# voidstrike/FPSG

Hardware: AMD Instinct MI355X
Metric: episodes/sec (+ Chamfer-kernel HBM GB/s in roofline.hbm), 2048-pt clouds, 224x224 images; episode = fwd + Chamfer + bwd, step = E episodes + all-reduce + Adam (higher is better)
Workload: dtype f32

## Files before the change

### fpsg_amd/_hip.py

```python
from __future__ import annotations

import ctypes
import os
import threading

import torch

_HERE = os.path.dirname(os.path.abspath(__file__))
LIB_PATH = os.environ.get("FPSG_HIP_LIB") or os.path.join(_HERE, "libfpsg_hip.so")

_c_f32p = ctypes.c_void_p
_c_i32p = ctypes.c_void_p
_c_int = ctypes.c_int
_c_stream = ctypes.c_void_p

SIGNATURES = {
    "fpsg_version": [],
    "fpsg_last_error": [],
    "fpsg_chamfer_fwd": [_c_f32p, _c_f32p, _c_int, _c_int, _c_int,
                         _c_f32p, _c_i32p, _c_f32p, _c_i32p, _c_stream],
    "fpsg_chamfer_bwd": [_c_f32p, _c_f32p, _c_i32p, _c_i32p, _c_f32p, _c_f32p,
                         _c_int, _c_int, _c_int, _c_f32p, _c_f32p, _c_stream],
    "fpsg_chamfer_losses": [_c_f32p, _c_f32p, _c_int, _c_int, _c_int, _c_int, ctypes.c_float, ctypes.c_float, _c_f32p,
                            _c_stream],
# ... 44 lines not shown
                                 _c_stream],
    "fpsg_sinkhorn_grad_workspace_floats": [_c_int, _c_int, _c_int],
    "fpsg_sinkhorn_divergence_grad": [_c_f32p, _c_f32p, _c_int, _c_int, _c_int, ctypes.c_void_p, _c_int, _c_f32p, _c_f32p,
                                      _c_f32p, _c_f32p, _c_stream],
    "fpsg_dec1_tiles": [_c_int],
    "fpsg_dec1_fits": [_c_int, _c_int, _c_int],
    "fpsg_dec1_fwd": [_c_f32p, _c_f32p, _c_int, _c_int, _c_f32p, _c_f32p, _c_f32p, _c_f32p, _c_f32p, _c_int, _c_int,
                      _c_int, _c_int, _c_int, ctypes.c_float, _c_f32p, _c_f32p, _c_f32p, _c_f32p, _c_stream],
    "fpsg_dec1_bwd": [_c_f32p, _c_f32p, _c_f32p, _c_int, _c_int, _c_f32p, _c_f32p, _c_int, _c_int, _c_int, _c_int,
                      _c_int, _c_f32p, _c_f32p, _c_f32p, _c_f32p, _c_f32p, _c_stream],
    "fpsg_dec1_fwd_ld": [_c_f32p, _c_int, _c_f32p, _c_int, _c_int, _c_f32p, _c_int, _c_f32p, _c_f32p, _c_f32p, _c_f32p, _c_int,
                         _c_int, _c_int, _c_int, _c_int, ctypes.c_float, _c_f32p, _c_int, _c_f32p, _c_f32p, _c_f32p,
                         _c_stream],
    "fpsg_dec1_bwd_ld": [_c_f32p, _c_int, _c_f32p, _c_int, _c_f32p, _c_int, _c_int, _c_f32p, _c_int, _c_f32p, _c_int, _c_int,
                         _c_int, _c_int, _c_int, _c_int, _c_f32p, _c_f32p, _c_f32p, _c_f32p, _c_f32p, _c_stream],
    "fpsg_bn_act_rows_fwd": [_c_f32p, _c_int, ctypes.POINTER(ctypes.c_int), ctypes.POINTER(ctypes.c_int), _c_int,
                             _c_f32p, _c_f32p, _c_f32p, _c_int, ctypes.c_float, _c_int, ctypes.c_float, _c_f32p,
                             _c_f32p, _c_f32p, _c_stream],
    "fpsg_bn_act_rows_bwd": [_c_f32p, _c_int, ctypes.POINTER(ctypes.c_int), ctypes.POINTER(ctypes.c_int), _c_int,
                             _c_f32p, _c_f32p, _c_f32p, _c_int, _c_int, ctypes.c_float, _c_f32p, _c_f32p, _c_f32p,
                             _c_f32p, _c_stream],
    "fpsg_bn_workspace_floats": [_c_int, _c_int, _c_int],
    "fpsg_bn_act_fwd": [_c_f32p, _c_f32p, _c_f32p, _c_f32p, _c_f32p, _c_f32p, ctypes.c_float, _c_int, _c_int, _c_int, _c_int,
                        ctypes.c_float, _c_int, ctypes.c_float, _c_f32p, _c_f32p, _c_f32p, _c_f32p, _c_f32p,
                        _c_stream],
    "fpsg_bn_act_bwd": [_c_f32p, _c_f32p, _c_f32p, _c_f32p, _c_int, _c_int, _c_int, _c_int, _c_int,
                        ctypes.c_float, _c_f32p, _c_f32p, _c_f32p, _c_f32p, _c_f32p, _c_f32p, _c_stream],
    "fpsg_bn_act_bwd_coef": [_c_f32p, _c_f32p, _c_f32p, _c_f32p, _c_int, _c_int, _c_int, _c_int, _c_int, ctypes.c_float,
                             _c_f32p, _c_f32p, _c_f32p, _c_f32p, _c_stream],
    "fpsg_bn_act_bwd_parts": [_c_f32p, _c_f32p, _c_f32p, _c_f32p, _c_int, _c_int, _c_int, _c_int, _c_int,
# ... 134 lines not shown
                         ctypes.POINTER(ctypes.c_float), _c_int, ctypes.c_void_p, ctypes.c_void_p, _c_f32p, _c_i32p,
                         _c_f32p, ctypes.c_void_p, ctypes.c_size_t, _c_stream],
    "fpsg_mesh_render_materials_workspace_bytes": [_c_int, _c_int, _c_int, _c_int, _c_int, _c_int, _c_int],
    "fpsg_mesh_render_materials": [_c_f32p, _c_int, _c_i32p, _c_int, _c_i32p, _c_f32p, ctypes.POINTER(ctypes.c_float),
                                   _c_int, ctypes.POINTER(ctypes.c_int32), _c_int, ctypes.c_void_p, ctypes.c_longlong,
                                   _c_f32p, _c_int, _c_int, _c_int, _c_int, ctypes.c_float,
                                   ctypes.POINTER(ctypes.c_float), _c_int, ctypes.c_void_p, ctypes.c_void_p, _c_f32p,
                                   _c_i32p, _c_f32p, ctypes.c_void_p, ctypes.c_size_t, _c_stream],
    "fpsg_points_render_workspace_bytes": [_c_int, _c_int, _c_int, _c_int, _c_int],
    "fpsg_points_render": [_c_f32p, ctypes.c_void_p, _c_int, _c_int, _c_f32p, _c_int, _c_int, _c_int, _c_int,
                           ctypes.c_float, ctypes.c_float, ctypes.POINTER(ctypes.c_float), _c_int, ctypes.c_void_p,
                           ctypes.c_void_p, _c_f32p, _c_i32p, _c_f32p, ctypes.c_void_p, ctypes.c_size_t, _c_stream],
}
_RESTYPES = {"fpsg_last_error": ctypes.c_char_p, "fpsg_grad_norm_workspace_bytes": ctypes.c_size_t,
"fpsg_chamfer_workspace_bytes": ctypes.c_size_t,
             "fpsg_sinkhorn_workspace_floats": ctypes.c_size_t,
             "fpsg_sinkhorn_grad_workspace_floats": ctypes.c_size_t,
             "fpsg_knn_workspace_floats": ctypes.c_size_t,
             "fpsg_bn_workspace_floats": ctypes.c_size_t, "fpsg_bn_pool_workspace_floats": ctypes.c_size_t, "fpsg_bn_max_workspace_floats": ctypes.c_size_t, "fpsg_bn_max_dz_offset": ctypes.c_size_t, "fpsg_conv_first_dw_workspace_floats": ctypes.c_size_t, "fpsg_emd_workspace_floats": ctypes.c_size_t, "fpsg_emd_exact_workspace_floats": ctypes.c_size_t, "fpsg_emd_cross_workspace_bytes": ctypes.c_size_t, "fpsg_occupancy_grid_workspace_bytes": ctypes.c_size_t, "fpsg_fps_workspace_bytes": ctypes.c_size_t, "fpsg_max_bwd_scatter_workspace_floats": ctypes.c_size_t,
             "fpsg_wino_dw_fused_workspace_floats": ctypes.c_size_t, "fpsg_gemm_split_workspace_floats": ctypes.c_size_t, "fpsg_gemm_split_packed_a_bytes": ctypes.c_size_t, "fpsg_edgeconv_stats_ws_floats": ctypes.c_size_t,
             "fpsg_repulsion_workspace_bytes": ctypes.c_size_t,
             "fpsg_expansion_workspace_bytes": ctypes.c_size_t,
             "fpsg_uniform_workspace_bytes": ctypes.c_size_t,
             "fpsg_swd_workspace_bytes": ctypes.c_size_t,
             "fpsg_mesh_cdf_workspace_bytes": ctypes.c_size_t,
             "fpsg_mesh_render_workspace_bytes": ctypes.c_size_t,
             "fpsg_mesh_render_materials_workspace_bytes": ctypes.c_size_t,
             "fpsg_points_render_workspace_bytes": ctypes.c_size_t}

_lib = None
# ... 53 lines not shown
```

### fpsg_amd/csrc/bnact.hip

```cpp
#include <algorithm>
#include <initializer_list>

#include "fpsg_common.h"

namespace fpsg {
namespace {

constexpr int kBnThreads = 256;
constexpr int kBnSeg = 4096;
constexpr int kBnSlices = 64;
constexpr int kBnU = kBnSeg / 4 / kBnThreads;

enum BnAct { kActNone = 0, kActRelu = 1, kActLeaky = 2 };

template <int ACT>
__device__ __forceinline__ float act_fwd(float z, float slope) {
  if (ACT == kActRelu) return z > 0.0f ? z : 0.0f;
  if (ACT == kActLeaky) return z > 0.0f ? z : z * slope;
  return z;
}
template <int ACT>
__device__ __forceinline__ float act_grad(float z, float slope) {
  if (ACT == kActRelu) return z > 0.0f ? 1.0f : 0.0f;
  if (ACT == kActLeaky) return z > 0.0f ? 1.0f : slope;
// ... 255 lines not shown
  for (int off = 32; off >= 1; off >>= 1) a += __shfl_down(a, off, 64);
  if (threadIdx.x == 0) dpb[c] = (float)a;
}

constexpr int kBnSmallMax = 16384;

constexpr int kBnMaxSegs = 4;
struct BnSegs {
  int ld;
  int off[kBnMaxSegs], len[kBnMaxSegs];
  int staged[kBnMaxSegs];
  int tpr_log2[kBnMaxSegs];
  int stat_stride;
};

template <int MODE, int ACT>
__global__ __launch_bounds__(kBnThreads) void bn_small_kernel(
    const float* __restrict__ x, const float* __restrict__ dy, const float* __restrict__ gamma,
    const float* __restrict__ beta, const float* __restrict__ pb, int N, int C, BnSegs segs, int training, float eps,
    float slope, float* __restrict__ out, float* __restrict__ chan, float* __restrict__ batch_mean,
    float* __restrict__ batch_var_unbiased, float* __restrict__ dgamma, float* __restrict__ dbeta,
    float* __restrict__ dpb, float* __restrict__ run_mean, float* __restrict__ run_var, float momentum) {
  const int sgi = blockIdx.y;
  const int L = segs.len[sgi], ld = segs.ld, staged = segs.staged[sgi], tpr_log2 = segs.tpr_log2[sgi];
  x += segs.off[sgi];
  out += segs.off[sgi];
  if (MODE == 1) dy += segs.off[sgi];
  chan += (size_t)sgi * 4 * C;
  if (batch_mean) batch_mean += (size_t)sgi * segs.stat_stride;
  if (batch_var_unbiased) batch_var_unbiased += (size_t)sgi * segs.stat_stride;
  if (MODE == 1) {
    dgamma += (size_t)sgi * C;
    dbeta += (size_t)sgi * C;
    if (dpb) dpb += (size_t)sgi * C;
  }
  extern __shared__ __attribute__((aligned(16))) float stage[];
  __shared__ float red[8];
  __shared__ float bc[4];
  const int c = blockIdx.x;
  const float b = pb ? pb[c] : 0.0f;
  const double count = (double)N * (double)L;
// ... 97 lines not shown
        chan[c] = bc[0]; chan[C + c] = bc[1]; chan[2 * C + c] = bc[2]; chan[3 * C + c] = bc[3];
        const float unbiased = (float)(count > 1.0 ? var * count / (count - 1.0) : var);
        if (batch_mean) batch_mean[c] = (float)mean;
        if (batch_var_unbiased) batch_var_unbiased[c] = unbiased;
        if (run_mean && momentum >= 0.0f) {
          run_mean[c] = fma_rn(momentum, (float)mean, (1.0f - momentum) * run_mean[c]);
          run_var[c] = fma_rn(momentum, unbiased, (1.0f - momentum) * run_var[c]);
        }
      } else {
        dbeta[c] = a0; dgamma[c] = a1;
        const double k2 = training ? -(double)sc * a1 * rs / count : 0.0;
        bc[0] = sc; bc[1] = (float)k2;
        bc[2] = training ? (float)(-(double)sc * a0 / count - k2 * mu) : 0.0f;
      }
    }
    __syncthreads();
    if (MODE == 0) { sc = bc[0]; sh = bc[1]; }
  } else {
    if (threadIdx.x == 0) { bc[0] = sc; bc[1] = 0.0f; bc[2] = 0.0f; }
    __syncthreads();
  }
  const float k1 = bc[0], k2 = bc[1], k3 = bc[2];
  float acc = 0.0f, unused = 0.0f;
  for (int n = n0; n < N; n += rpi) {
    const size_t base = ((size_t)n * C + c) * ld;
    if (vec) {
      const v4f* __restrict__ xp = reinterpret_cast<const v4f*>(x + base);
      const v4f* __restrict__ gp = reinterpret_cast<const v4f*>(MODE == 1 ? dy + base : x + base);
      v4f* __restrict__ op = reinterpret_cast<v4f*>(out + base);
      for (int e = e0; e < L4; e += tpr) {
// ... 645 lines not shown
  g.ld = ld;
  for (int i = 0; i < nseg; ++i) {
    FPSG_REQUIRE(seg_len[i] > 0 && seg_len[i] <= kBnSmallMax && seg_off[i] >= 0 && seg_off[i] + seg_len[i] <= ld,
                 FPSG_E_SHAPE, "%s: segment %d = [%d, +%d) does not fit a row of %d (a segment holds at most %d)", fn, i,
                 seg_off[i], seg_len[i], ld, kBnSmallMax);
    FPSG_REQUIRE((seg_off[i] & 3) == 0, FPSG_E_ALIGN, "%s: segment offset %d must be a multiple of 4", fn, seg_off[i]);
    for (int j = 0; j < i; ++j)
      FPSG_REQUIRE(seg_off[i] >= seg_off[j] + seg_len[j] || seg_off[j] >= seg_off[i] + seg_len[i], FPSG_E_SHAPE,
                   "%s: segments %d and %d overlap", fn, j, i);
    small_segment(g, i, 1, seg_off[i], seg_len[i], 1, backward);
  }
  return 0;
}

}
}

extern "C" size_t fpsg_bn_workspace_floats(int N, int C, int L) {
  if (N <= 0 || C <= 0 || L <= 0) return 0;
  return fpsg::plain_workspace(N, C, L).floats;
}

extern "C" int fpsg_bn_act_fwd(const float* x, const float* pre_bias, const float* gamma, const float* beta,
                               float* running_mean, float* running_var, float momentum, int N, int C, int L,
                               int training, float eps, int act, float slope, float* y, float* chan,
                               float* batch_mean, float* batch_var_unbiased, float* ws, fpsg_stream_t stream) {
  using namespace fpsg;
  const char* fn = "fpsg_bn_act_fwd";
  int rc = check_dims(fn, N, C, L, act);
  if (rc) return rc;
// ... 248 lines not shown
```

### fpsg_amd/csrc/decoder.hip

```cpp
#include "fpsg_common.h"

namespace fpsg {
namespace {

constexpr int kD1Waves = 8;
constexpr int kD1Threads = 64 * kD1Waves;
constexpr int kD1ChPerWave = 4;
constexpr int kD1Tile = kD1Waves * kD1ChPerWave;
constexpr int kD1MaxBP = 8192;
constexpr size_t kD1MaxLds = 160 * 1024;

inline size_t dec1_lds_bytes(int B, int P, bool bwd) {
  return ((size_t)3 * B * P + (size_t)kD1Tile * B + (bwd ? (size_t)kD1Waves * 64 * 12 : 0)) * sizeof(float);
}

__device__ __forceinline__ double wave_sum_f64(double v) {
#pragma unroll
  for (int m = 1; m < 64; m <<= 1) {
    const unsigned long long u = (unsigned long long)__double_as_longlong(v);
    unsigned lo = (unsigned)u, hi = (unsigned)(u >> 32);
    lo = (unsigned)__shfl_xor((int)lo, m, 64);
    hi = (unsigned)__shfl_xor((int)hi, m, 64);
    v += __longlong_as_double((long long)(((unsigned long long)hi << 32) | lo));
  }
// ... 291 lines not shown
    }
  }
}

inline int dec1_check(const char* fn, int G, int D, int B, int P, int ldw, int wofs, bool bwd) {
  FPSG_REQUIRE(G > 0 && D > 0 && B > 0 && P > 0, FPSG_E_SHAPE, "%s: G,D,B,P must be positive (got %d,%d,%d,%d)", fn, G,
               D, B, P);
  FPSG_REQUIRE(P % 4 == 0 && P <= 256 && ((P / 4) & (P / 4 - 1)) == 0, FPSG_E_SHAPE,
               "%s: P = %d must be 4 x a power of two, at most 256 (lanes of 4 points, a cloud = one lane group)", fn, P);
  FPSG_REQUIRE((long)B * P <= kD1MaxBP, FPSG_E_LIMIT, "%s: B*P = %ld exceeds %d (the patch's points live in LDS)", fn,
               (long)B * P, kD1MaxBP);
  FPSG_REQUIRE(dec1_lds_bytes(B, P, bwd) <= kD1MaxLds, FPSG_E_LIMIT,
               "%s: B = %d, P = %d need %zu bytes of LDS, more than the %zu of a CU", fn, B, P, dec1_lds_bytes(B, P, bwd),
               kD1MaxLds);
  FPSG_REQUIRE(G <= 65535 && wofs >= 0 && wofs + 3 <= ldw, FPSG_E_SHAPE, "%s: bad G / weight columns", fn);
  return 0;
}

}
}

extern "C" int fpsg_dec1_tiles(int D) { return (D + fpsg::kD1Tile - 1) / fpsg::kD1Tile; }

extern "C" int fpsg_dec1_fits(int B, int P, int bwd) {
  return fpsg::dec1_check("fpsg_dec1_fits", 1, 1, B, P, 3, 0, bwd != 0) == 0;
}

extern "C" int fpsg_dec1_fwd_ld(const float* hlat, int ld_hlat, const float* w, int ldw, int wofs, const float* pts, int ld_pts,
                                const float* gamma, const float* beta, const float* running_mean,
                                const float* running_var, int G, int D, int B, int P, int training, float eps,
// ... 57 lines not shown
                                       hipFuncAttributeMaxDynamicSharedMemorySize, (int)lds_bytes);
    if (e != hipSuccess) { set_error("fpsg_dec1_bwd: %s", hipGetErrorString(e)); return (int)e; }
  }
  hipLaunchKernelGGL(kern, dim3((unsigned)fpsg_dec1_tiles(D), (unsigned)G), dim3(kD1Threads), lds_bytes,
                     static_cast<hipStream_t>(stream), a, dout, chan, dhlat, dw, dpts_part, dgamma, dbeta);
  return launch_status("fpsg_dec1_bwd");
}

extern "C" int fpsg_dec1_bwd(const float* dout, const float* hlat, const float* w, int ldw, int wofs,
                             const float* pts, const float* chan, int G, int D, int B, int P, int training,
                             float* dhlat, float* dw, float* dpts_part, float* dgamma, float* dbeta,
                             fpsg_stream_t stream) {
  return fpsg_dec1_bwd_ld(dout, B * P, hlat, B, w, ldw, wofs, pts, B * P, chan, G, D, B, P, training, 0, dhlat, dw,
                          dpts_part, dgamma, dbeta, stream);
}
```

### fpsg_amd/csrc/fpsg_common.h

```cpp
#pragma once
#include <hip/hip_runtime.h>
#include <stdint.h>
#include <stdio.h>

#include "../../include/fpsg_hip.h"

namespace fpsg {

void set_error(const char* fmt, ...);

inline bool misaligned4(const void* p) { return (reinterpret_cast<uintptr_t>(p) & 3u) != 0; }

inline int launch_status(const char* what) {
  hipError_t e = hipGetLastError();
  if (e != hipSuccess) {
    set_error("%s: %s", what, hipGetErrorString(e));
    return static_cast<int>(e);
  }
  return 0;
}

#define FPSG_REQUIRE_PTR(p)                                   \
  do {                                                        \
    if ((p) == nullptr) {                                     \
// ... 88 lines not shown
```

### fpsg_amd/point_cloud_net.py

```python
from __future__ import annotations

import os

import torch
import torch.nn as nn
import torch.nn.functional as F

from . import bn_counters
from .fused_bn import batch_norm_act, batch_norm_act_rows, bn_act
from .pointnet import PointNetfeat
from .utils import get_template


def get_activation(argument: str):
    table = {
        "relu": F.relu,
        "sigmoid": torch.sigmoid,
        "softplus": F.softplus,
        "logsigmoid": F.logsigmoid,
        "softsign": F.softsign,
        "tanh": torch.tanh,
    }
    if argument not in table:
        raise ValueError(f"Invalid activation: {argument}")
# ... 313 lines not shown
            for i, Bi in enumerate(batches):
                part = torch.empty((G, T, 3, Bi * P), dtype=torch.float32, device=dev)
                rc = lib.fpsg_dec1_bwd_ld(_hip.ptr(dout) + 4 * b0 * P, M, _hip.ptr(hlat) + 4 * b0, B, _hip.ptr(w1), K, L,
                                          _hip.ptr(pts) + 4 * b0 * P, M, _hip.ptr(chan[i]), G, D, Bi, P, 1,
                                          1 if i else 0, _hip.ptr(dhlat) + 4 * b0, _hip.ptr(gw), _hip.ptr(part),
                                          _hip.ptr(dgamma), _hip.ptr(dbeta), _hip.stream_of(x))
                _hip.check(rc, "fpsg_dec1_bwd_ld")
                torch.sum(part, dim=1, out=gpts[:, :, b0 * P:(b0 + Bi) * P])
                b0 += Bi
        torch.bmm(dhlat, x.unsqueeze(0).expand(G, B, L), out=gw[..., :L])
        gb = dhlat.sum(dim=2, keepdim=True)
        gx = torch.matmul(dhlat.reshape(G * D, B).t(), w1.reshape(G * D, K)[:, :L])
        return gw, gb, gx, gpts, dgamma, dbeta, None, None, None


class _StackFrozen(torch.autograd.Function):

    @staticmethod
    def forward(ctx, key, *tensors):
        from . import winograd
        cache = winograd.frozen_cache()
        full_key = ("stack", key) + tuple(t.data_ptr() for t in tensors)
        if cache is not None and full_key in cache:
            return cache[full_key].detach()
        out = torch.stack([t.detach() for t in tensors])
        if cache is not None:
            cache[full_key] = out
            return out.detach()
        return out

# ... 311 lines not shown
        else:
            cols = []
            for i, b in enumerate(batches):
                if grids[i] is not None:
                    g = torch.stack([t for per_cluster in grids[i] for t in per_cluster])
                else:
                    g = torch.empty((G, b, dim, P), dtype=torch.float32, device=x.device)
                    g = g.uniform_(0, 1, generator=generator) if square else g.normal_(0, 1, generator=generator)
                cols.append(g.permute(0, 2, 1, 3).reshape(G, g.size(2), b * P))
            h = torch.cat(cols, dim=2)

        defs = [c.deformer for c in clusters]
        w, b = pack["d1"]
        h = _group_batch_norm_rows(torch.bmm(w, h), [d.bn1 for d in defs], R, act, pack["dbn1"], b.reshape(-1), seg_lens)
        w, b = pack["d2"]
        h = _group_batch_norm_rows(torch.bmm(w, h), [d.bn2 for d in defs], R, act, pack["dbn2"], b.reshape(-1), seg_lens)
        w, b = pack["d3"]
        pts = torch.tanh(torch.baddbmm(b, w, h))

        nodes = [n for c in clusters for n in c.node_pool]
        w1, b1 = pack["n1"]
        if w1.size(2) - self.conf.raw_dim != L:
            raise ValueError(f"PCDecoder: hidden size {L} does not match the first layer ({w1.size(2) - self.conf.raw_dim} latent columns)")
        bn1s = [n.bn1 for n in nodes]
        gamma, beta = pack["nbn1"]
        h, stats = _DecoderLayer1Pair.apply(w1, b1, x, pts, gamma, beta, bn1s[0].eps, P, batches)
        with torch.no_grad():
            _update_running_calls(bn1s, 1, stats)
        w, b = pack["n2"]
        h = _group_batch_norm_rows(_bmm_wide(w, h), [n.bn2 for n in nodes], 1, act, pack["nbn2"], b.reshape(-1), seg_lens)
        w, b = pack["n3"]
        h = _group_batch_norm_rows(_bmm_wide(w, h), [n.bn3 for n in nodes], 1, act, pack["nbn3"], b.reshape(-1), seg_lens)
        w, b = pack["n4"]
        out = torch.tanh(torch.baddbmm(b, w, h))
        return out.view(G, 3, B, P).permute(2, 0, 3, 1).reshape(B, G * P, 3).contiguous()

    def pack_parameters(self):
        if not self.batched:
            return None
        cache = key = None
        if not torch.is_grad_enabled() and os.environ.get("FPSG_EVAL_PACK_CACHE", "1") != "0":
            from . import winograd
            cache = winograd.frozen_cache()
            first = next(self.parameters())
            key = ("decoder_pack", id(self), first.data_ptr(), first.device)
            if cache is not None and key in cache:
                return cache[key]
        pack = self._build_pack()
        if cache is not None and not (first.is_cuda and torch.cuda.is_current_stream_capturing()):
# ... 44 lines not shown
        act = clusters[0].deformer.activation
        if grid is None:
            dim = clusters[0].template[0].dim
            if type(clusters[0].template[0]).__name__ == "SquareTemplate":
                g = torch.empty((G, B, dim, P), dtype=torch.float32, device=x.device).uniform_(0, 1, generator=generator)
            else:
                g = torch.empty((G, B, dim, P), dtype=torch.float32, device=x.device).normal_(0, 1, generator=generator)
        else:
            g = torch.stack([t for per_cluster in grid for t in per_cluster])
        h = g.permute(0, 2, 1, 3).reshape(G, g.size(2), B * P)

        defs = [c.deformer for c in clusters]
        w, b = pack["d1"]
        h = _group_batch_norm(torch.bmm(w, h), [d.bn1 for d in defs], R, act, pack["dbn1"], b.reshape(-1))
        w, b = pack["d2"]
        h = _group_batch_norm(torch.bmm(w, h), [d.bn2 for d in defs], R, act, pack["dbn2"], b.reshape(-1))
        w, b = pack["d3"]
        pts = torch.tanh(torch.baddbmm(b, w, h))

        nodes = [n for c in clusters for n in c.node_pool]
        w1, b1 = pack["n1"]
        D = w1.size(1)
        if w1.size(2) - self.conf.raw_dim != L:
            raise ValueError(f"PCDecoder: hidden size {L} does not match the first layer ({w1.size(2) - self.conf.raw_dim} latent columns)")
        bn1s = [n.bn1 for n in nodes]
        if self.conf.raw_dim == 3 and _layer1_fused_ok(x, pts, B, P, act):
            gamma, beta = pack["nbn1"]
            training = bn1s[0].training
            rm = rv = None
            if not training:
                rm = torch.stack([b_.running_mean for b_ in bn1s]).reshape(-1)
                rv = torch.stack([b_.running_var for b_ in bn1s]).reshape(-1)
            h, bmean, bvar = _DecoderLayer1.apply(w1, b1, x, pts, gamma, beta, rm, rv, training, bn1s[0].eps, P)
            if training:
                with torch.no_grad():
                    _update_running(bn1s, 1, bmean, bvar)
        else:
            w_lat, w_pts, b = pack["n1_split"]() if callable(pack["n1_split"]) else pack["n1_split"]
            h_lat = torch.matmul(w_lat, x.t()) + b
            h = torch.bmm(w_pts, pts).view(G, D, B, P) + h_lat.unsqueeze(-1)
            h = _group_batch_norm(h.view(G, D, B * P), bn1s, 1, act, pack["nbn1"])
        w, b = pack["n2"]
        h = _group_batch_norm(_bmm_wide(w, h), [n.bn2 for n in nodes], 1, act, pack["nbn2"], b.reshape(-1))
        w, b = pack["n3"]
        h = _group_batch_norm(_bmm_wide(w, h), [n.bn3 for n in nodes], 1, act, pack["nbn3"], b.reshape(-1))
        w, b = pack["n4"]
        out = torch.tanh(torch.baddbmm(b, w, h))
        return out.view(G, 3, B, P).permute(2, 0, 3, 1).reshape(B, G * P, 3).contiguous()
```

### include/fpsg_hip.h

```cpp
#ifndef FPSG_HIP_H
#define FPSG_HIP_H

#include <stddef.h>
#include <stdint.h>

#ifdef __cplusplus
extern "C" {
#endif

typedef void* fpsg_stream_t;

#define FPSG_ABI_VERSION 1

#define FPSG_E_NULL   (-1)
#define FPSG_E_SHAPE  (-2)
#define FPSG_E_ALIGN  (-3)
#define FPSG_E_LIMIT  (-4)

int         fpsg_version(void);
const char* fpsg_last_error(void);

int fpsg_chamfer_fwd(const float* xyz1, const float* xyz2, int B, int N, int M,
                     float* dist1, int32_t* idx1, float* dist2, int32_t* idx2,
                     fpsg_stream_t stream);
// ... 175 lines not shown
                  const float* gamma, const float* beta, const float* running_mean, const float* running_var,
                  int G, int D, int B, int P, int training, float eps, float* out, float* chan,
                  float* batch_mean, float* batch_var_unbiased, fpsg_stream_t stream);
int fpsg_dec1_bwd(const float* dout, const float* hlat, const float* w, int ldw, int wofs, const float* pts,
                  const float* chan, int G, int D, int B, int P, int training, float* dhlat, float* dw,
                  float* dpts_part, float* dgamma, float* dbeta, fpsg_stream_t stream);

int fpsg_dec1_fwd_ld(const float* hlat, int ld_hlat, const float* w, int ldw, int wofs, const float* pts, int ld_pts,
                     const float* gamma, const float* beta, const float* running_mean, const float* running_var,
                     int G, int D, int B, int P, int training, float eps, float* out, int ld_out, float* chan,
                     float* batch_mean, float* batch_var_unbiased, fpsg_stream_t stream);
int fpsg_dec1_bwd_ld(const float* dout, int ld_dout, const float* hlat, int ld_hlat, const float* w, int ldw, int wofs,
                     const float* pts, int ld_pts, const float* chan, int G, int D, int B, int P, int training,
                     int accumulate, float* dhlat, float* dw, float* dpts_part, float* dgamma, float* dbeta,
                     fpsg_stream_t stream);

size_t fpsg_bn_workspace_floats(int N, int C, int L);
int fpsg_bn_act_fwd(const float* x, const float* pre_bias, const float* gamma, const float* beta,
                    float* running_mean, float* running_var, float momentum, int N, int C, int L, int training,
                    float eps, int act, float slope, float* y, float* chan, float* batch_mean,
                    float* batch_var_unbiased, float* ws, fpsg_stream_t stream);
int fpsg_bn_stats(const float* x, const float* pre_bias, const float* gamma, const float* beta,
                  float* running_mean, float* running_var, float momentum, int N, int C, int L, int training,
                  float eps, float* chan, float* batch_mean, float* batch_var_unbiased, float* ws,
                  const float* parts, int n_parts, fpsg_stream_t stream);
int fpsg_bn_act_bwd(const float* x, const float* pre_bias, const float* dy, const float* chan, int N, int C,
                    int L, int training, int act, float slope, float* dx, float* dgamma, float* dbeta,
                    float* dpre_bias, float* coef, float* ws, fpsg_stream_t stream);
int fpsg_bn_act_bwd_coef(const float* x, const float* pre_bias, const float* dy, const float* chan, int N, int C,
                         int L, int training, int act, float slope, float* dgamma, float* dbeta, float* coef,
// ... 183 lines not shown
```

Baseline: 46.05.

## Fuse decoder tail batch-norm, activation, final projection and tanh into custom kernels

Adds fused HIP kernels for the last decoder stage. The forward computes batch-norm stats, then applies BN, ReLU, the small J-output projection, bias and tanh, writing directly into the final permuted output layout. A matching backward fuses the tanh derivative, the dz/dw/db reductions and the BN input gradient using LDS staging. The aim is to avoid materialising the normalised hidden activation, plus the separate baddbmm, tanh and permute/contiguous passes. The trade-off is extra code paths, gated on training and grad mode, and a row length limit for LDS.

```diff
diff --git a/fpsg_amd/_hip.py b/fpsg_amd/_hip.py
--- a/fpsg_amd/_hip.py
+++ b/fpsg_amd/_hip.py
@@ -82,6 +82,15 @@
                          _c_stream],
     "fpsg_dec1_bwd_ld": [_c_f32p, _c_int, _c_f32p, _c_int, _c_f32p, _c_int, _c_int, _c_f32p, _c_int, _c_f32p, _c_int, _c_int,
                          _c_int, _c_int, _c_int, _c_int, _c_f32p, _c_f32p, _c_f32p, _c_f32p, _c_f32p, _c_stream],
+    "fpsg_dec_tail_fits": [_c_int, _c_int, _c_int, _c_int, _c_int, _c_int, _c_int],
+    "fpsg_dec_tail_ws_floats": [_c_int, _c_int, _c_int],
+    "fpsg_dec_tail_fwd": [_c_f32p, _c_int, ctypes.POINTER(ctypes.c_int), ctypes.POINTER(ctypes.c_int), _c_int, _c_f32p,
+                          _c_f32p, _c_f32p, _c_f32p, _c_f32p, _c_int, _c_int, _c_int, ctypes.c_float, _c_int, _c_f32p,
+                          _c_int, _c_int, _c_int, _c_int, _c_int, ctypes.c_long, _c_f32p, _c_f32p, _c_stream],
+    "fpsg_dec_tail_bwd": [_c_f32p, _c_int, ctypes.POINTER(ctypes.c_int), ctypes.POINTER(ctypes.c_int), _c_int, _c_f32p,
+                          _c_f32p, _c_f32p, _c_f32p, _c_f32p, _c_int, _c_int, _c_int, _c_int, _c_int, ctypes.c_long,
+                          _c_int, _c_int, _c_int, _c_int, _c_f32p, _c_f32p, _c_f32p, _c_f32p, _c_f32p, _c_f32p, _c_f32p,
+                          _c_stream],
     "fpsg_bn_act_rows_fwd": [_c_f32p, _c_int, ctypes.POINTER(ctypes.c_int), ctypes.POINTER(ctypes.c_int), _c_int,
                              _c_f32p, _c_f32p, _c_f32p, _c_int, ctypes.c_float, _c_int, ctypes.c_float, _c_f32p,
                              _c_f32p, _c_f32p, _c_stream],
@@ -246,6 +255,7 @@
 }
 _RESTYPES = {"fpsg_last_error": ctypes.c_char_p, "fpsg_grad_norm_workspace_bytes": ctypes.c_size_t,
 "fpsg_chamfer_workspace_bytes": ctypes.c_size_t,
+             "fpsg_dec_tail_ws_floats": ctypes.c_size_t,
              "fpsg_sinkhorn_workspace_floats": ctypes.c_size_t,
              "fpsg_sinkhorn_grad_workspace_floats": ctypes.c_size_t,
              "fpsg_knn_workspace_floats": ctypes.c_size_t,
diff --git a/fpsg_amd/csrc/bnact.hip b/fpsg_amd/csrc/bnact.hip
--- a/fpsg_amd/csrc/bnact.hip
+++ b/fpsg_amd/csrc/bnact.hip
@@ -293,7 +293,7 @@
   int stat_stride;
 };
 
-template <int MODE, int ACT>
+template <int MODE, int ACT, bool APPLY = true>
 __global__ __launch_bounds__(kBnThreads) void bn_small_kernel(
     const float* __restrict__ x, const float* __restrict__ dy, const float* __restrict__ gamma,
     const float* __restrict__ beta, const float* __restrict__ pb, int N, int C, BnSegs segs, int training, float eps,
@@ -301,9 +301,9 @@
     float* __restrict__ batch_var_unbiased, float* __restrict__ dgamma, float* __restrict__ dbeta,
     float* __restrict__ dpb, float* __restrict__ run_mean, float* __restrict__ run_var, float momentum) {
   const int sgi = blockIdx.y;
-  const int L = segs.len[sgi], ld = segs.ld, staged = segs.staged[sgi], tpr_log2 = segs.tpr_log2[sgi];
+  const int L = segs.len[sgi], ld = segs.ld, staged = APPLY ? segs.staged[sgi] : 0, tpr_log2 = segs.tpr_log2[sgi];
   x += segs.off[sgi];
-  out += segs.off[sgi];
+  if (APPLY) out += segs.off[sgi];
   if (MODE == 1) dy += segs.off[sgi];
   chan += (size_t)sgi * 4 * C;
   if (batch_mean) batch_mean += (size_t)sgi * segs.stat_stride;
@@ -431,6 +431,7 @@
         bc[2] = training ? (float)(-(double)sc * a0 / count - k2 * mu) : 0.0f;
       }
     }
+    if (!APPLY) return;
     __syncthreads();
     if (MODE == 0) { sc = bc[0]; sh = bc[1]; }
   } else {
@@ -1106,6 +1107,20 @@
 }
 
 }
+
+int bn_rows_stats(const char* fn, const float* x, int ld, const int* seg_off, const int* seg_len, int nseg,
+                  const float* pre_bias, const float* gamma, const float* beta, int C, float eps, float* chan,
+                  float* stats, hipStream_t s) {
+  BnSegs g;
+  int rc = rows_segments(fn, ld, seg_off, seg_len, nseg, C, kActNone, false, g);
+  if (rc) return rc;
+  g.stat_stride = 2 * C;
+  hipLaunchKernelGGL((bn_small_kernel<0, kActNone, false>), dim3(C, nseg), dim3(kBnThreads), 0, s, x, nullptr, gamma,
+                     beta, pre_bias, 1, C, g, 1, eps, 0.0f, nullptr, chan, stats, stats ? stats + C : nullptr, nullptr,
+                     nullptr, nullptr, nullptr, nullptr, -1.0f);
+  return launch_status(fn);
+}
+
 }
 
 extern "C" size_t fpsg_bn_workspace_floats(int N, int C, int L) {
diff --git a/fpsg_amd/csrc/decoder.hip b/fpsg_amd/csrc/decoder.hip
--- a/fpsg_amd/csrc/decoder.hip
+++ b/fpsg_amd/csrc/decoder.hip
@@ -329,6 +329,280 @@
                "%s: B = %d, P = %d need %zu bytes of LDS, more than the %zu of a CU", fn, B, P, dec1_lds_bytes(B, P, bwd),
                kD1MaxLds);
   FPSG_REQUIRE(G <= 65535 && wofs >= 0 && wofs + 3 <= ldw, FPSG_E_SHAPE, "%s: bad G / weight columns", fn);
+  return 0;
+}
+
+constexpr int kTailMaxJ = 4;
+constexpr int kTailMaxSegs = 4;
+constexpr int kTailSegMax = 16384;
+constexpr int kTailWaves = 8;
+constexpr int kTailFwdThreads = 64 * kTailWaves;
+constexpr int kTailCols = 256;
+constexpr int kTailU = 4;
+constexpr int kTailBwdThreads = 256;
+
+struct TailSegs {
+  int ld, nseg;
+  int off[kTailMaxSegs], len[kTailMaxSegs];
+  int tile0[kTailMaxSegs + 1];
+};
+struct TailLayout { int sg, sj, sb, sp, P; };
+
+template <int ACT> __device__ __forceinline__ float tail_act(float z) { return ACT == 1 ? (z > 0.0f ? z : 0.0f) : z; }
+template <int ACT> __device__ __forceinline__ float tail_mask(float z) { return ACT == 1 ? (z > 0.0f ? 1.0f : 0.0f) : 1.0f; }
+
+__device__ __forceinline__ v4f tail_load4(const float* __restrict__ p, int n) {
+  if (n >= 4) return *reinterpret_cast<const v4f*>(p);
+  v4f v = {0.0f, 0.0f, 0.0f, 0.0f};
+  if (n > 0) v[0] = p[0];
+  if (n > 1) v[1] = p[1];
+  if (n > 2) v[2] = p[2];
+  return v;
+}
+
+template <int ACT, int J>
+__global__ __launch_bounds__(kTailFwdThreads) void dec_tail_fwd_kernel(
+    const float* __restrict__ x, const float* __restrict__ pb, const float* __restrict__ chan,
+    const float* __restrict__ w, const float* __restrict__ bias, TailSegs segs, int C, int GC, TailLayout lay,
+    float* __restrict__ out) {
+  __shared__ __attribute__((aligned(16))) float red[kTailWaves][J][kTailCols];
+  const int g = blockIdx.y;
+  int s = 0;
+  for (int i = 1; i < segs.nseg; ++i)
+    if ((int)blockIdx.x >= segs.tile0[i]) s = i;
+  const int L = segs.len[s], ld = segs.ld;
+  const int t0 = ((int)blockIdx.x - segs.tile0[s]) * kTailCols;
+  const int tid = threadIdx.x, lane = tid & 63;
+  const int wave = __builtin_amdgcn_readfirstlane(tid >> 6);
+  const int col = t0 + lane * 4;
+  const int nval = L - col;
+  const float* __restrict__ ch = chan + (size_t)s * 4 * GC;
+  const float* __restrict__ xg = x + (size_t)g * C * ld + segs.off[s] + col;
+  float acc[J][4];
+#pragma unroll
+  for (int j = 0; j < J; ++j)
+#pragma unroll
+    for (int k = 0; k < 4; ++k) acc[j][k] = 0.0f;
+  for (int c0 = wave; c0 < C; c0 += kTailWaves * kTailU) {
+    v4f xq[kTailU];
+#pragma unroll
+    for (int u = 0; u < kTailU; ++u) {
+      const int c = c0 + u * kTailWaves;
+      xq[u] = (v4f){0.0f, 0.0f, 0.0f, 0.0f};
+      if (c < C) xq[u] = tail_load4(xg + (size_t)c * ld, nval);
+    }
+#pragma unroll
+    for (int u = 0; u < kTailU; ++u) {
+      const int c = c0 + u * kTailWaves;
+      if (c < C) {
+        const int gc = g * C + c;
+        const float bv = pb ? pb[gc] : 0.0f, sc = ch[gc], sh = ch[GC + gc];
+        float wj[J];
+#pragma unroll
+        for (int j = 0; j < J; ++j) wj[j] = w[((size_t)g * J + j) * C + c];
+#pragma unroll
+        for (int k = 0; k < 4; ++k) {
+          const float a = tail_act<ACT>(fma_rn(xq[u][k] + bv, sc, sh));
+#pragma unroll
+          for (int j = 0; j < J; ++j) acc[j][k] = fma_rn(wj[j], a, acc[j][k]);
+        }
+      }
+    }
+  }
+#pragma unroll
+  for (int j = 0; j < J; ++j)
+    *reinterpret_cast<v4f*>(&red[wave][j][lane * 4]) = (v4f){acc[j][0], acc[j][1], acc[j][2], acc[j][3]};
+  __syncthreads();
+  for (int i = tid; i < J * kTailCols; i += kTailFwdThreads) {
+    const int j = i / kTailCols, cl = i - j * kTailCols;
+    if (t0 + cl >= L) continue;
+    float sum = red[0][j][cl];
+#pragma unroll
+    for (int v = 1; v < kTailWaves; ++v) sum += red[v][j][cl];
+    const int q = segs.off[s] + t0 + cl;
+    const int qb = q / lay.P, qp = q - qb * lay.P;
+    out[(size_t)g * lay.sg + (size_t)j * lay.sj + (size_t)qb * lay.sb + (size_t)qp * lay.sp] =
+        tanhf(sum + bias[g * J + j]);
+  }
+}
+
+__global__ __launch_bounds__(256) void dec_tail_dt_kernel(const float* __restrict__ out, const float* __restrict__ gout,
+                                                          TailLayout lay, int J, int Q, int ldt,
+                                                          float* __restrict__ dt) {
+  const int g = blockIdx.y;
+  const int q = blockIdx.x * 256 + threadIdx.x;
+  if (q >= Q) return;
+  const int qb = q / lay.P, qp = q - qb * lay.P;
+  const size_t base = (size_t)g * lay.sg + (size_t)qb * lay.sb + (size_t)qp * lay.sp;
+  for (int j = 0; j < J; ++j) {
+    const float o = out[base + (size_t)j * lay.sj];
+    dt[((size_t)g * J + j) * ldt + q] = gout[base + (size_t)j * lay.sj] * (1.0f - o * o);
+  }
+}
+
+template <int N>
+__device__ __forceinline__ void tail_block_sum(float (&v)[N], float* red ) {
+#pragma unroll
+  for (int i = 0; i < N; ++i)
+#pragma unroll
+    for (int off = 32; off >= 1; off >>= 1) v[i] += __shfl_down(v[i], off, 64);
+  const int wave = threadIdx.x >> 6, lane = threadIdx.x & 63;
+  if (lane == 0) {
+#pragma unroll
+    for (int i = 0; i < N; ++i) red[wave * N + i] = v[i];
+  }
+  __syncthreads();
+  if (threadIdx.x == 0) {
+#pragma unroll
+    for (int i = 0; i < N; ++i) v[i] = (red[i] + red[N + i]) + (red[2 * N + i] + red[3 * N + i]);
+  }
+}
+
+template <int ACT, int J>
+__global__ __launch_bounds__(kTailBwdThreads) void dec_tail_bwd_kernel(
+    const float* __restrict__ x, const float* __restrict__ pb, const float* __restrict__ chan,
+    const float* __restrict__ w, const float* __restrict__ dt, TailSegs segs, int C, int GC,
+    float* __restrict__ dx, float* __restrict__ dgamma, float* __restrict__ dbeta, float* __restrict__ dpb,
+    float* __restrict__ dw, float* __restrict__ db) {
+  extern __shared__ __attribute__((aligned(16))) float stage[];
+  constexpr int NV = 2 + 2 * J;
+  __shared__ float red[4 * NV];
+  __shared__ float bc[3];
+  const int s = blockIdx.y, gc = blockIdx.x;
+  const int g = gc / C, c = gc - g * C, G = GC / C;
+  const int L = segs.len[s], ld = segs.ld, L4 = (L + 3) >> 2;
+  const int tid = threadIdx.x;
+  const float* __restrict__ ch = chan + (size_t)s * 4 * GC;
+  const float sc = ch[gc], sh = ch[GC + gc], mu = ch[2 * GC + gc], rs = ch[3 * GC + gc];
+  const float bv = pb ? pb[gc] : 0.0f;
+  float wj[J];
+#pragma unroll
+  for (int j = 0; j < J; ++j) wj[j] = w[((size_t)g * J + j) * C + c];
+  const float* __restrict__ xr = x + (size_t)gc * ld + segs.off[s];
+  const float* __restrict__ dtr = dt + (size_t)g * J * ld + segs.off[s];
+  float* __restrict__ dxr = dx + (size_t)gc * ld + segs.off[s];
+  v4f* __restrict__ sx = reinterpret_cast<v4f*>(stage);
+  v4f* __restrict__ sd = sx + L4;
+  float v[NV];
+#pragma unroll
+  for (int i = 0; i < NV; ++i) v[i] = 0.0f;
+  for (int e0 = tid; e0 < L4; e0 += kTailBwdThreads * kTailU) {
+    v4f xq[kTailU], tq[kTailU][J];
+#pragma unroll
+    for (int u = 0; u < kTailU; ++u) {
+      const int e = e0 + u * kTailBwdThreads;
+      xq[u] = (v4f){0.0f, 0.0f, 0.0f, 0.0f};
+#pragma unroll
+      for (int j = 0; j < J; ++j) tq[u][j] = xq[u];
+      if (e < L4) {
+        xq[u] = tail_load4(xr + 4 * e, L - 4 * e);
+#pragma unroll
+        for (int j = 0; j < J; ++j) tq[u][j] = tail_load4(dtr + (size_t)j * ld + 4 * e, L - 4 * e);
+      }
+    }
+#pragma unroll
+    for (int u = 0; u < kTailU; ++u) {
+      const int e = e0 + u * kTailBwdThreads;
+      if (e < L4) {
+        const int n = L - 4 * e;
+        v4f xv = xq[u], dz;
+#pragma unroll
+        for (int k = 0; k < 4; ++k) {
+          xv[k] += bv;
+          const float z = fma_rn(xv[k], sc, sh);
+          const float a = tail_act<ACT>(z);
+          float t = wj[0] * tq[u][0][k];
+#pragma unroll
+          for (int j = 1; j < J; ++j) t = fma_rn(wj[j], tq[u][j][k], t);
+          dz[k] = k < n ? t * tail_mask<ACT>(z) : 0.0f;
+          v[0] += dz[k];
+          v[1] = fma_rn(dz[k], (xv[k] - mu) * rs, v[1]);
+#pragma unroll
+          for (int j = 0; j < J; ++j) {
+            v[2 + j] = fma_rn(tq[u][j][k], a, v[2 + j]);
+            v[2 + J + j] += tq[u][j][k];
+          }
+        }
+        sx[e] = xv;
+        sd[e] = dz;
+      }
+    }
+  }
+  tail_block_sum<NV>(v, red);
+  if (tid == 0) {
+    const double count = (double)L;
+    dbeta[(size_t)s * GC + gc] = v[0];
+    dgamma[(size_t)s * GC + gc] = v[1];
+    const double k2 = -(double)sc * v[1] * rs / count;
+    bc[0] = sc; bc[1] = (float)k2;
+    bc[2] = (float)(-(double)sc * v[0] / count - k2 * mu);
+#pragma unroll
+    for (int j = 0; j < J; ++j) {
+      dw[(((size_t)s * G + g) * J + j) * C + c] = v[2 + j];
+      if (c == 0) db[((size_t)s * G + g) * J + j] = v[2 + J + j];
+    }
+  }
+  __syncthreads();
+  const float k1 = bc[0], k2 = bc[1], k3 = bc[2];
+  float acc[1] = {0.0f};
+  for (int e = tid; e < L4; e += kTailBwdThreads) {
+    const v4f xv = sx[e], dz = sd[e];
+    v4f r;
+#pragma unroll
+    for (int k = 0; k < 4; ++k) r[k] = fma_rn(k1, dz[k], fma_rn(k2, xv[k], k3));
+    const int n = L - 4 * e;
+    if (n >= 4) {
+      *reinterpret_cast<v4f*>(dxr + 4 * e) = r;
+      acc[0] += (r[0] + r[1]) + (r[2] + r[3]);
+    } else {
+      for (int k = 0; k < n; ++k) { dxr[4 * e + k] = r[k]; acc[0] += r[k]; }
+    }
+  }
+  if (dpb) {
+    __syncthreads();
+    tail_block_sum<1>(acc, red);
+    if (tid == 0) dpb[(size_t)s * GC + gc] = acc[0];
+  }
+}
+
+inline size_t tail_bwd_lds(int max_len) { return (size_t)2 * ((max_len + 3) / 4) * sizeof(v4f); }
+
+inline int dec_tail_check(const char* fn, int G, int C, int J, int ld, const int* seg_off, const int* seg_len, int nseg,
+                          int act, const TailLayout* lay, long elems, TailSegs& t) {
+  FPSG_REQUIRE(G > 0 && G <= 65535 && C > 0 && (long)G * C <= 0x7fffffffL / 4, FPSG_E_SHAPE,
+               "%s: G, C must be positive, G <= 65535, G*C < 2^29 (got %d, %d)", fn, G, C);
+  FPSG_REQUIRE(J >= 1 && J <= kTailMaxJ, FPSG_E_LIMIT, "%s: J = %d outputs (1..%d)", fn, J, kTailMaxJ);
+  FPSG_REQUIRE(act == 0 || act == 1, FPSG_E_SHAPE, "%s: activation %d (0 none, 1 ReLU)", fn, act);
+  FPSG_REQUIRE(nseg >= 1 && nseg <= kTailMaxSegs, FPSG_E_LIMIT, "%s: %d segments (1..%d)", fn, nseg, kTailMaxSegs);
+  FPSG_REQUIRE(seg_off != nullptr && seg_len != nullptr, FPSG_E_NULL, "%s: null segment arrays", fn);
+  FPSG_REQUIRE(ld > 0 && (ld & 3) == 0, FPSG_E_ALIGN, "%s: ld = %d must be a positive multiple of 4", fn, ld);
+  FPSG_REQUIRE((long)G * J * ld <= 0x7fffffffL, FPSG_E_LIMIT, "%s: G*J*ld = %ld exceeds 2^31 - 1", fn, (long)G * J * ld);
+  t = TailSegs{};
+  t.ld = ld;
+  t.nseg = nseg;
+  int qmax = 0;
+  for (int i = 0; i < nseg; ++i) {
+    FPSG_REQUIRE(seg_len[i] > 0 && seg_len[i] <= kTailSegMax && seg_off[i] >= 0 && seg_off[i] <= ld - seg_len[i],
+                 FPSG_E_SHAPE, "%s: segment %d = [%d, +%d) does not fit a row of %d (a segment holds at most %d)", fn, i,
+                 seg_off[i], seg_len[i], ld, kTailSegMax);
+    FPSG_REQUIRE((seg_off[i] & 3) == 0, FPSG_E_ALIGN, "%s: segment offset %d must be a multiple of 4", fn, seg_off[i]);
+    for (int j = 0; j < i; ++j)
+      FPSG_REQUIRE(seg_off[i] >= seg_off[j] + seg_len[j] || seg_off[j] >= seg_off[i] + seg_len[i], FPSG_E_SHAPE,
+                   "%s: segments %d and %d overlap", fn, j, i);
+    t.off[i] = seg_off[i];
+    t.len[i] = seg_len[i];
+    t.tile0[i + 1] = t.tile0[i] + (seg_len[i] + kTailCols - 1) / kTailCols;
+    qmax = qmax > seg_off[i] + seg_len[i] - 1 ? qmax : seg_off[i] + seg_len[i] - 1;
+  }
+  if (lay) {
+    FPSG_REQUIRE(lay->P > 0 && lay->sg >= 0 && lay->sj >= 0 && lay->sb >= 0 && lay->sp >= 0, FPSG_E_SHAPE,
+                 "%s: P must be positive and the strides of out non-negative", fn);
+    const int pmax = qmax < lay->P ? qmax : lay->P - 1;
+    const long last = (long)(G - 1) * lay->sg + (long)(J - 1) * lay->sj + (long)(qmax / lay->P) * lay->sb +
+                      (long)pmax * lay->sp;
+    FPSG_REQUIRE(last < elems, FPSG_E_SHAPE, "%s: the last element addressed (%ld) lies outside out (%ld elements)", fn,
+                 last, elems);
+  }
   return 0;
 }
 
@@ -416,3 +690,97 @@
   return fpsg_dec1_bwd_ld(dout, B * P, hlat, B, w, ldw, wofs, pts, B * P, chan, G, D, B, P, training, 0, dhlat, dw,
                           dpts_part, dgamma, dbeta, stream);
 }
+
+extern "C" int fpsg_dec_tail_fits(int G, int C, int J, int ld, int nseg, int max_seg_len, int act) {
+  using namespace fpsg;
+  if (nseg < 1 || nseg > kTailMaxSegs) return 0;
+  int off[kTailMaxSegs], len[kTailMaxSegs];
+  const int first = (max_seg_len + 3) / 4 * 4;
+  for (int i = 0; i < nseg; ++i) { off[i] = i ? first + 4 * (i - 1) : 0; len[i] = i ? 1 : max_seg_len; }
+  TailSegs t;
+  if (max_seg_len <= 0 || dec_tail_check("fpsg_dec_tail_fits", G, C, J, ld, off, len, nseg, act, nullptr, 0, t)) return 0;
+  return tail_bwd_lds(max_seg_len) <= kD1MaxLds ? 1 : 0;
+}
+
+extern "C" size_t fpsg_dec_tail_ws_floats(int G, int J, int ld) {
+  if (G <= 0 || J <= 0 || ld <= 0) return 0;
+  return (size_t)G * J * ld;
+}
+
+extern "C" int fpsg_dec_tail_fwd(const float* x, int ld, const int* seg_off, const int* seg_len, int nseg,
+                                 const float* pre_bias, const float* gamma, const float* beta, const float* w,
+                                 const float* b, int G, int C, int J, float eps, int act, float* out, int out_sg,
+                                 int out_sj, int out_sb, int out_sp, int P, long out_elems, float* chan, float* stats,
+                                 fpsg_stream_t stream) {
+  using namespace fpsg;
+  const char* fn = "fpsg_dec_tail_fwd";
+  TailSegs t;
+  const TailLayout lay{out_sg, out_sj, out_sb, out_sp, P};
+  int rc = dec_tail_check(fn, G, C, J, ld, seg_off, seg_len, nseg, act, &lay, out_elems, t);
+  if (rc) return rc;
+  FPSG_REQUIRE_PTR(x); FPSG_REQUIRE_PTR(gamma); FPSG_REQUIRE_PTR(beta); FPSG_REQUIRE_PTR(w); FPSG_REQUIRE_PTR(b);
+  FPSG_REQUIRE_PTR(out); FPSG_REQUIRE_PTR(chan);
+  FPSG_REQUIRE((reinterpret_cast<uintptr_t>(x) & 15) == 0, FPSG_E_ALIGN, "%s: x must be 16-byte aligned", fn);
+  hipStream_t s = static_cast<hipStream_t>(stream);
+  if ((rc = bn_rows_stats(fn, x, ld, seg_off, seg_len, nseg, pre_bias, gamma, beta, G * C, eps, chan, stats, s))) return rc;
+  const dim3 grid((unsigned)t.tile0[nseg], (unsigned)G);
+#define FPSG_TAIL_FWD(A, JJ) hipLaunchKernelGGL((dec_tail_fwd_kernel<A, JJ>), grid, dim3(kTailFwdThreads), 0, s, x, \
+                                                pre_bias, chan, w, b, t, C, G * C, lay, out)
+#define FPSG_TAIL_FWD_J(A) \
+  switch (J) { case 1: FPSG_TAIL_FWD(A, 1); break; case 2: FPSG_TAIL_FWD(A, 2); break; \
+               case 3: FPSG_TAIL_FWD(A, 3); break; default: FPSG_TAIL_FWD(A, 4); break; }
+  if (act == 1) { FPSG_TAIL_FWD_J(1) } else { FPSG_TAIL_FWD_J(0) }
+#undef FPSG_TAIL_FWD_J
+#undef FPSG_TAIL_FWD
+  return launch_status(fn);
+}
+
+extern "C" int fpsg_dec_tail_bwd(const float* x, int ld, const int* seg_off, const int* seg_len, int nseg,
+                                 const float* pre_bias, const float* w, const float* chan, const float* out,
+                                 const float* gout, int out_sg, int out_sj, int out_sb, int out_sp, int P,
+                                 long out_elems, int G, int C, int J, int act, float* dx, float* dgamma, float* dbeta,
+                                 float* dpre_bias, float* dw, float* db, float* ws, fpsg_stream_t stream) {
+  using namespace fpsg;
+  const char* fn = "fpsg_dec_tail_bwd";
+  TailSegs t;
+  const TailLayout lay{out_sg, out_sj, out_sb, out_sp, P};
+  int rc = dec_tail_check(fn, G, C, J, ld, seg_off, seg_len, nseg, act, &lay, out_elems, t);
+  if (rc) return rc;
+  FPSG_REQUIRE_PTR(x); FPSG_REQUIRE_PTR(w); FPSG_REQUIRE_PTR(chan); FPSG_REQUIRE_PTR(out); FPSG_REQUIRE_PTR(gout);
+  FPSG_REQUIRE_PTR(dx); FPSG_REQUIRE_PTR(dgamma); FPSG_REQUIRE_PTR(dbeta); FPSG_REQUIRE_PTR(dw); FPSG_REQUIRE_PTR(db);
+  FPSG_REQUIRE_PTR(ws);
+  FPSG_REQUIRE((reinterpret_cast<uintptr_t>(x) & 15) == 0 && (reinterpret_cast<uintptr_t>(dx) & 15) == 0 &&
+                   (reinterpret_cast<uintptr_t>(ws) & 15) == 0,
+               FPSG_E_ALIGN, "%s: x, dx and ws must be 16-byte aligned", fn);
+  int max_len = 0, Q = 0;
+  for (int i = 0; i < nseg; ++i) {
+    max_len = max_len > seg_len[i] ? max_len : seg_len[i];
+    Q = Q > seg_off[i] + seg_len[i] ? Q : seg_off[i] + seg_len[i];
+  }
+  const size_t lds_bytes = tail_bwd_lds(max_len);
+  FPSG_REQUIRE(lds_bytes <= kD1MaxLds, FPSG_E_LIMIT, "%s: a segment of %d columns needs %zu bytes of LDS, more than the %zu of a CU",
+               fn, max_len, lds_bytes, kD1MaxLds);
+  hipStream_t s = static_cast<hipStream_t>(stream);
+  hipLaunchKernelGGL(dec_tail_dt_kernel, dim3((unsigned)((Q + 255) / 256), (unsigned)G), dim3(256), 0, s, out, gout, lay,
+                     J, Q, ld, ws);
+  if ((rc = launch_status(fn))) return rc;
+  const dim3 grid((unsigned)(G * C), (unsigned)nseg);
+#define FPSG_TAIL_BWD(A, JJ)                                                                                          \
+  do {                                                                                                                \
+    auto kern = dec_tail_bwd_kernel<A, JJ>;                                                                           \
+    if (lds_bytes > 65536) {                                                                                          \
+      hipError_t e = hipFuncSetAttribute(reinterpret_cast<const void*>(kern),                                         \
+                                         hipFuncAttributeMaxDynamicSharedMemorySize, (int)lds_bytes);                 \
+      if (e != hipSuccess) { set_error("%s: %s", fn, hipGetErrorString(e)); return (int)e; }                          \
+    }                                                                                                                 \
+    hipLaunchKernelGGL(kern, grid, dim3(kTailBwdThreads), lds_bytes, s, x, pre_bias, chan, w, (const float*)ws, t, C, \
+                       G * C, dx, dgamma, dbeta, dpre_bias, dw, db);                                                  \
+  } while (0)
+#define FPSG_TAIL_BWD_J(A) \
+  switch (J) { case 1: FPSG_TAIL_BWD(A, 1); break; case 2: FPSG_TAIL_BWD(A, 2); break; \
+               case 3: FPSG_TAIL_BWD(A, 3); break; default: FPSG_TAIL_BWD(A, 4); break; }
+  if (act == 1) { FPSG_TAIL_BWD_J(1) } else { FPSG_TAIL_BWD_J(0) }
+#undef FPSG_TAIL_BWD_J
+#undef FPSG_TAIL_BWD
+  return launch_status(fn);
+}
diff --git a/fpsg_amd/csrc/fpsg_common.h b/fpsg_amd/csrc/fpsg_common.h
--- a/fpsg_amd/csrc/fpsg_common.h
+++ b/fpsg_amd/csrc/fpsg_common.h
@@ -8,6 +8,10 @@
 namespace fpsg {
 
 void set_error(const char* fmt, ...);
+
+int bn_rows_stats(const char* fn, const float* x, int ld, const int* seg_off, const int* seg_len, int nseg,
+                  const float* pre_bias, const float* gamma, const float* beta, int C, float eps, float* chan,
+                  float* stats, hipStream_t s);
 
 inline bool misaligned4(const void* p) { return (reinterpret_cast<uintptr_t>(p) & 3u) != 0; }
 
diff --git a/fpsg_amd/point_cloud_net.py b/fpsg_amd/point_cloud_net.py
--- a/fpsg_amd/point_cloud_net.py
+++ b/fpsg_amd/point_cloud_net.py
@@ -351,6 +351,90 @@
         return gw, gb, gx, gpts, dgamma, dbeta, None, None, None
 
 
+def _tail_fused_ok(x, w, seg_lens, act) -> bool:
+    from . import _hip, fused_bn
+    if not (x.is_cuda and x.dtype == torch.float32 and act is F.relu and fused_bn.fused_enabled()
+            and os.environ.get("FPSG_DECODER_TAIL", "1") != "0"):
+        return False
+    G, C, M = x.shape
+    if M % 4 or any(n % 4 for n in seg_lens[:-1]) or sum(seg_lens) != M:
+        return False
+    return _hip.load().fpsg_dec_tail_fits(G, C, w.shape[1], M, len(seg_lens), max(seg_lens), 1) != 0
+
+
+class _DecoderTail(torch.autograd.Function):
+
+    @staticmethod
+    def forward(ctx, x, pre_bias, gamma, beta, w, b, seg_lens, eps, P):
+        import ctypes
+        from . import _hip
+        lib = _hip.load()
+        G, C, M = x.shape
+        J = w.shape[1]
+        seg_lens = [int(n) for n in seg_lens]
+        nseg = len(seg_lens)
+        offs = [sum(seg_lens[:i]) for i in range(nseg)]
+        c_off, c_len = (ctypes.c_int * nseg)(*offs), (ctypes.c_int * nseg)(*seg_lens)
+        dev = x.device
+        ctx.set_materialize_grads(False)
+        x, w = x.contiguous(), w.contiguous()
+        bias = b.reshape(G, J).contiguous()
+        if P:
+            out = torch.empty((M // P, G * P, J), dtype=torch.float32, device=dev)
+            lay = (P * J, 1, G * P * J, J, P)
+        else:
+            out = torch.empty((G, J, M), dtype=torch.float32, device=dev)
+            lay = (J * M, M, 0, 1, M)
+        chan = torch.empty((nseg, 4, G * C), dtype=torch.float32, device=dev)
+        stats = torch.empty((nseg, 2, G * C), dtype=torch.float32, device=dev)
+        with torch.cuda.device(dev):
+            rc = lib.fpsg_dec_tail_fwd(_hip.ptr(x), M, c_off, c_len, nseg, _hip.ptr(pre_bias), _hip.ptr(gamma),
+                                       _hip.ptr(beta), _hip.ptr(w), _hip.ptr(bias), G, C, J, float(eps), 1, _hip.ptr(out),
+                                       *lay, out.numel(), _hip.ptr(chan), _hip.ptr(stats), _hip.stream_of(x))
+        _hip.check(rc, "fpsg_dec_tail_fwd")
+        ctx.save_for_backward(x, pre_bias, w, chan, out)
+        ctx.cfg = (G, C, J, M, offs, seg_lens, lay, tuple(b.shape))
+        ctx.mark_non_differentiable(stats)
+        return out, stats
+
+    @staticmethod
+    def backward(ctx, gout, _gstats):
+        if gout is None:
+            return (None,) * 9
+        import ctypes
+        from . import _hip
+        lib = _hip.load()
+        x, pre_bias, w, chan, out = ctx.saved_tensors
+        G, C, J, M, offs, seg_lens, lay, b_shape = ctx.cfg
+        nseg = len(seg_lens)
+        c_off, c_len = (ctypes.c_int * nseg)(*offs), (ctypes.c_int * nseg)(*seg_lens)
+        dev = x.device
+        gout = gout.contiguous()
+        dx = torch.empty_like(x)
+        grads = torch.empty((3, nseg, G * C), dtype=torch.float32, device=dev)
+        dw = torch.empty((nseg, G, J, C), dtype=torch.float32, device=dev)
+        db = torch.empty((nseg,) + b_shape, dtype=torch.float32, device=dev)
+        ws = torch.empty((lib.fpsg_dec_tail_ws_floats(G, J, M),), dtype=torch.float32, device=dev)
+        with torch.cuda.device(dev):
+            rc = lib.fpsg_dec_tail_bwd(_hip.ptr(x), M, c_off, c_len, nseg, _hip.ptr(pre_bias), _hip.ptr(w), _hip.ptr(chan),
+                                       _hip.ptr(out), _hip.ptr(gout), *lay, out.numel(), G, C, J, 1, _hip.ptr(dx),
+                                       _hip.ptr(grads[0]), _hip.ptr(grads[1]), _hip.ptr(grads[2]), _hip.ptr(dw),
+                                       _hip.ptr(db), _hip.ptr(ws), _hip.stream_of(x))
+        _hip.check(rc, "fpsg_dec_tail_bwd")
+        if nseg > 1:
+            g, dw, db = grads.sum(1), dw.sum(0), db.sum(0)
+        else:
+            g, dw, db = grads[:, 0], dw[0], db[0]
+        return dx, g[2], g[0], g[1], dw, db, None, None, None
+
+
+def _decoder_tail(h, bns, calls_per_bn, affine, pre_bias, w, b, seg_lens, P):
+    out, stats = _DecoderTail.apply(h, pre_bias, affine[0], affine[1], w, b, tuple(seg_lens), bns[0].eps, P)
+    with torch.no_grad():
+        _update_running_calls(bns, calls_per_bn, stats)
+    return out
+
+
 class _StackFrozen(torch.autograd.Function):
 
     @staticmethod
@@ -692,9 +776,13 @@
         w, b = pack["d1"]
         h = _group_batch_norm_rows(torch.bmm(w, h), [d.bn1 for d in defs], R, act, pack["dbn1"], b.reshape(-1), seg_lens)
         w, b = pack["d2"]
-        h = _group_batch_norm_rows(torch.bmm(w, h), [d.bn2 for d in defs], R, act, pack["dbn2"], b.reshape(-1), seg_lens)
-        w, b = pack["d3"]
-        pts = torch.tanh(torch.baddbmm(b, w, h))
+        w3, b3 = pack["d3"]
+        h = torch.bmm(w, h)
+        if _tail_fused_ok(h, w3, seg_lens, act):
+            pts = _decoder_tail(h, [d.bn2 for d in defs], R, pack["dbn2"], b.reshape(-1), w3, b3, seg_lens, 0)
+        else:
+            h = _group_batch_norm_rows(h, [d.bn2 for d in defs], R, act, pack["dbn2"], b.reshape(-1), seg_lens)
+            pts = torch.tanh(torch.baddbmm(b3, w3, h))
 
         nodes = [n for c in clusters for n in c.node_pool]
         w1, b1 = pack["n1"]
@@ -708,9 +796,12 @@
         w, b = pack["n2"]
         h = _group_batch_norm_rows(_bmm_wide(w, h), [n.bn2 for n in nodes], 1, act, pack["nbn2"], b.reshape(-1), seg_lens)
         w, b = pack["n3"]
-        h = _group_batch_norm_rows(_bmm_wide(w, h), [n.bn3 for n in nodes], 1, act, pack["nbn3"], b.reshape(-1), seg_lens)
-        w, b = pack["n4"]
-        out = torch.tanh(torch.baddbmm(b, w, h))
+        w4, b4 = pack["n4"]
+        h = _bmm_wide(w, h)
+        if _tail_fused_ok(h, w4, seg_lens, act):
+            return _decoder_tail(h, [n.bn3 for n in nodes], 1, pack["nbn3"], b.reshape(-1), w4, b4, seg_lens, P)
+        h = _group_batch_norm_rows(h, [n.bn3 for n in nodes], 1, act, pack["nbn3"], b.reshape(-1), seg_lens)
+        out = torch.tanh(torch.baddbmm(b4, w4, h))
         return out.view(G, 3, B, P).permute(2, 0, 3, 1).reshape(B, G * P, 3).contiguous()
 
     def pack_parameters(self):
@@ -785,9 +876,14 @@
         w, b = pack["d1"]
         h = _group_batch_norm(torch.bmm(w, h), [d.bn1 for d in defs], R, act, pack["dbn1"], b.reshape(-1))
         w, b = pack["d2"]
-        h = _group_batch_norm(torch.bmm(w, h), [d.bn2 for d in defs], R, act, pack["dbn2"], b.reshape(-1))
-        w, b = pack["d3"]
-        pts = torch.tanh(torch.baddbmm(b, w, h))
+        w3, b3 = pack["d3"]
+        h = torch.bmm(w, h)
+        tail = defs[0].bn2.training and torch.is_grad_enabled()
+        if tail and _tail_fused_ok(h, w3, (B * P,), act):
+            pts = _decoder_tail(h, [d.bn2 for d in defs], R, pack["dbn2"], b.reshape(-1), w3, b3, (B * P,), 0)
+        else:
+            h = _group_batch_norm(h, [d.bn2 for d in defs], R, act, pack["dbn2"], b.reshape(-1))
+            pts = torch.tanh(torch.baddbmm(b3, w3, h))
 
         nodes = [n for c in clusters for n in c.node_pool]
         w1, b1 = pack["n1"]
@@ -814,7 +910,10 @@
         w, b = pack["n2"]
         h = _group_batch_norm(_bmm_wide(w, h), [n.bn2 for n in nodes], 1, act, pack["nbn2"], b.reshape(-1))
         w, b = pack["n3"]
-        h = _group_batch_norm(_bmm_wide(w, h), [n.bn3 for n in nodes], 1, act, pack["nbn3"], b.reshape(-1))
-        w, b = pack["n4"]
-        out = torch.tanh(torch.baddbmm(b, w, h))
+        w4, b4 = pack["n4"]
+        h = _bmm_wide(w, h)
+        if nodes[0].bn3.training and torch.is_grad_enabled() and _tail_fused_ok(h, w4, (B * P,), act):
+            return _decoder_tail(h, [n.bn3 for n in nodes], 1, pack["nbn3"], b.reshape(-1), w4, b4, (B * P,), P)
+        h = _group_batch_norm(h, [n.bn3 for n in nodes], 1, act, pack["nbn3"], b.reshape(-1))
+        out = torch.tanh(torch.baddbmm(b4, w4, h))
         return out.view(G, 3, B, P).permute(2, 0, 3, 1).reshape(B, G * P, 3).contiguous()
diff --git a/include/fpsg_hip.h b/include/fpsg_hip.h
--- a/include/fpsg_hip.h
+++ b/include/fpsg_hip.h
@@ -213,6 +213,18 @@
                      const float* pts, int ld_pts, const float* chan, int G, int D, int B, int P, int training,
                      int accumulate, float* dhlat, float* dw, float* dpts_part, float* dgamma, float* dbeta,
                      fpsg_stream_t stream);
+
+int fpsg_dec_tail_fits(int G, int C, int J, int ld, int nseg, int max_seg_len, int act);
+size_t fpsg_dec_tail_ws_floats(int G, int J, int ld);
+int fpsg_dec_tail_fwd(const float* x, int ld, const int* seg_off, const int* seg_len, int nseg,
+                      const float* pre_bias, const float* gamma, const float* beta, const float* w, const float* b,
+                      int G, int C, int J, float eps, int act, float* out, int out_sg, int out_sj, int out_sb,
+                      int out_sp, int P, long out_elems, float* chan, float* stats, fpsg_stream_t stream);
+int fpsg_dec_tail_bwd(const float* x, int ld, const int* seg_off, const int* seg_len, int nseg,
+                      const float* pre_bias, const float* w, const float* chan, const float* out, const float* gout,
+                      int out_sg, int out_sj, int out_sb, int out_sp, int P, long out_elems, int G, int C, int J,
+                      int act, float* dx, float* dgamma, float* dbeta, float* dpre_bias, float* dw, float* db,
+                      float* ws, fpsg_stream_t stream);
 
 size_t fpsg_bn_workspace_floats(int N, int C, int L);
 int fpsg_bn_act_fwd(const float* x, const float* pre_bias, const float* gamma, const float* beta,
```

Result: no change. 46.33, median of 6 (+0.6%).
